# filthyrake/telescope_cam_detection

Measured on AMD Instinct MI355X. Metric: frames_per_sec, higher is better.
Workload: dtype f16x3; 1 GPU; RT-DETR-R50 640x640 bs=8/GPU, uint8 BGR frames resident in HBM -> [8,300,6] detections in HBM; synthetic seeded weights; global_batch=8, parallelism=camera-shard x1, streams_per_gpu=1, batches_in_flight_per_gpu=1, hip_graph=True

## Files before the change

### telescope_cam_detection_amd/csrc/common.h

```cpp
#pragma once
#include <hip/hip_runtime.h>
#include <stdint.h>
#include <string.h>

#include <stdexcept>
#include <string>
#include <tuple>
#include <type_traits>
#include <utility>
#include <vector>

#include "error.h"

namespace rtd {

enum DType : int { BF16 = 0, F32 = 1, U8 = 2, I32 = 3, F16X2 = 4 };
constexpr int SPLIT_GROUP = 32;
enum Act : int { ACT_NONE = 0, ACT_RELU = 1, ACT_SILU = 2, ACT_GELU = 3, ACT_LRELU = 4  };
enum ResMode : int { RES_NONE = 0, RES_PRE = 1, RES_POST = 2 };
enum DecMethod : int { DEC_DEFAULT = 0, DEC_DISCRETE = 1 };

inline size_t dtype_size(int dt) { return dt == BF16 ? 2 : (dt == U8 ? 1 : 4); }

typedef __bf16 bf16;
// ... 67 lines not shown
template <typename... KArgs, typename... Args>
inline void rtd_launch(void (*kernel)(KArgs...), dim3 grid, dim3 block, unsigned shmem, hipStream_t s, Args&&... args) {
  static_assert(sizeof...(KArgs) == sizeof...(Args), "rtd_launch: argument count differs from the kernel's parameter count");
  ++t_launches;
  if (GraphBuild* gb = t_graph_build) {
    std::tuple<std::remove_cv_t<KArgs>...> vals{static_cast<KArgs>(std::forward<Args>(args))...};
    void* ptrs[sizeof...(KArgs) + 1];
    std::apply([&](auto&... v) { size_t i = 0; ((ptrs[i++] = (void*)&v), ...); (void)i; }, vals);
    gb->add_kernel((void*)kernel, grid, block, shmem, ptrs, s);
  } else {
    hipLaunchKernelGGL(kernel, grid, block, shmem, s, static_cast<KArgs>(std::forward<Args>(args))...);
  }
}

struct ConvOpts {
  int conv_mode = 0;
  int glds_min_blocks = 4;
  int glds_min_n = 128;
  int ws2_min_blocks = 257;
  int ws64_max_blocks = 160;
  int reg_epilogue = 1;
  int conv_reg = 3;
  int prefetch = 1;
  int split_ws2_min_blocks = 257;
  int split_ws64_max_blocks = 160;
  int split_flex = 1;
  int split_flex_min_nk = 4;
  int split_flex_small_max = 200;
  int split_sx = 3;
  int split_k2 = 1;
  int split_wsq = 1;
  int split_wsq_min_blocks = 257;
  int split_wsq_min_nk = 24;
};
ConvOpts& conv_opts_template();
bool conv_set_option(const char* name, int value);

struct ConvWorkspace {
  float* slab = nullptr;
  size_t slab_bytes = 0;
};

struct ConvArgs {
  Tensor x;
  const void* w;
  const float* bias;
  Tensor res;
  Tensor x2;
  int x_up2 = 0;
  const void* next_w = nullptr;
  const float* next_bias = nullptr;
  Tensor next_y;
  int next_kpad = 0, next_act = ACT_NONE;
  Tensor avg_y;
  int y_dead = 0;
  int prefer256 = 0;
  const ConvOpts* opts = nullptr;
  Tensor y;
  int KH = 1, KW = 1, stride = 1, pad = 0;
  int Kpad = 0, Npad = 0;
  int act = ACT_NONE, res_mode = RES_NONE;
  ConvWorkspace ws;
  const void* pf = nullptr;
  size_t pf_bytes = 0;
};
void launch_conv(const ConvArgs& a, hipStream_t s);
// ... 21 lines not shown
                      float eps, hipStream_t s);
void launch_add(const Tensor& a, const Tensor& b, const Tensor& y, hipStream_t s);
void launch_axpby(float alpha, const Tensor& a, const Tensor& b, const Tensor& y, hipStream_t s);
void launch_maxpool3x3s2(const Tensor& x, const Tensor& y, hipStream_t s);
void launch_upsample2x(const Tensor& x, const Tensor& y, hipStream_t s);
void launch_avgpool2(const Tensor& x, const Tensor& y, hipStream_t s);
void launch_attention(const Tensor& qk, const Tensor& v, const Tensor& o, int heads, hipStream_t s);
void launch_set_rows(const Tensor& y, const int32_t* rows, int nrows, int rows_per_image, const float* vec,
                     hipStream_t s);
void launch_rowmax(const Tensor& x, float* out, hipStream_t s);
void launch_topk(const float* keys, int B, int N, int K, int32_t* idx, float* vals, hipStream_t s);
void launch_gather_rows(const Tensor& src, const int32_t* idx, int rows_per_image, const Tensor& dst, hipStream_t s);
void launch_ref_init(const Tensor& boxdelta, const float* anchors, const int32_t* idx, int S, float* ref_unact8,
                     float* ref8, hipStream_t s);
void launch_msdeform(const Tensor& value, int value_coff, const Tensor& offaw, const float* ref8, const Tensor& out,
                     int heads, int hd, int n_levels, int n_points, const int32_t* level_hw_start, float offset_scale,
                     int method, hipStream_t s);
void launch_box_refine(const Tensor& delta, float* ref8, hipStream_t s);
void launch_postprocess_scores(const Tensor& logits, float* scores, hipStream_t s);
bool postprocess_fused_supported(const Tensor& logits, int B, int Q);
void launch_postprocess_fused(const Tensor& logits, const float* ref8, const float* scale_wh, int B, int Q, float* block6, hipStream_t s);
void launch_postprocess_gather(const float* topv, const int32_t* topi, const float* ref8, const float* scale_wh,
                               int B, int Q, int C, float* block6, hipStream_t s);
constexpr int RTD_MAX_BATCH = 64;
struct FrameArgs {
  const uint8_t* ptr[RTD_MAX_BATCH];
  float scale_wh[2 * RTD_MAX_BATCH];
  int n;
};
void launch_preprocess_identity(const FrameArgs& fa, int H, int W, const Tensor& y, float* scale_wh_dev, hipStream_t s);
void launch_set_scale(const FrameArgs& fa, float* scale_wh_dev, hipStream_t s);
void launch_set_frame_table(const FrameArgs& fa, const uint8_t** table_dev, float* scale_wh_dev, hipStream_t s);
void launch_stem0_u8(const uint8_t* const* table_dev, int n, int H, int W, const void* w, int Kpad, const float* bias, const Tensor& y, int act,
                     hipStream_t s);
struct ResizeCoef {
  const int32_t* hb;
  const int32_t* hk;
  const int32_t* vb;
  const int32_t* vk;
  int hks, vks;
};
void launch_resize_pil(const uint8_t* src, int sh, int sw, uint8_t* tmp, const Tensor& y, int image, const ResizeCoef& coef,
                       hipStream_t s);
void launch_u8_hwc_to_chw_f32(const uint8_t* src, int H, int W, float* out, hipStream_t s);
void launch_resize_pil_u8(const uint8_t* src, int sh, int sw, uint8_t* tmp, uint8_t* dst, int dh, int dw, const ResizeCoef& c, hipStream_t s);
struct DecLin {
  const float* w;
  const float* b;
  int ldw, N, K;
};
struct DecLN {
  const float* g;
  const float* b;
};

struct DecArgs {
  int mode;
  int attn_split;
  int split;
  int B, Q, D, heads, S, n_levels, n_points, ffn, C;
  float offset_scale;
  int method;
  const float* q_in;
  const float* kfrag_in;
  const float* vfrag_in;
  const float* hs_in;
  float* hs_out;
// ... 143 lines not shown
```

### telescope_cam_detection_amd/csrc/conv_igemm.hip

```cpp
#include <stdlib.h>
#include <string.h>

#include <algorithm>
#include <type_traits>

#include "common.h"

namespace rtd {

struct ConvK {
  const void* x = nullptr;
  const void* w = nullptr;
  const float* bias = nullptr;
  const void* res = nullptr;
  void* y = nullptr;
  int M = 0, H = 0, W = 0, Cin = 0;
  long long ldx = 0, x_bstride = 0;
  int OH = 0, OW = 0, OHW = 0;
  int N = 0, Kreal = 0, Kpad = 0;
  int KH = 1, KW = 1, stride = 1, pad = 0;
  long long ldy = 0, y_bstride = 0, ldr = 0, r_bstride = 0;
  int act = ACT_NONE, res_mode = RES_NONE, y_f32 = 0, res_f32 = 0;
  int ntn = 1;
  const void* pf = nullptr;
// ... 1690 lines not shown
    const long long rpix = (long long)b * a.r_bstride + (long long)p * a.ldr;
    if (a.res_split) split_load8((const sp16*)a.res, rpix, c, rv);
    else {
      const f32x4 t0 = *(const f32x4*)((const float*)a.res + rpix + c), t1 = *(const f32x4*)((const float*)a.res + rpix + c + 4);
#pragma unroll
      for (int e = 0; e < 4; ++e) { rv[e] = t0[e]; rv[4 + e] = t1[e]; }
    }
  }
#pragma unroll
  for (int e = 0; e < 8; ++e) {
    if (a.res_mode == RES_PRE) v[e] += rv[e];
    v[e] = act_fn(v[e], a.act);
    if (a.res_mode == RES_POST) v[e] += rv[e];
  }
  if (a.y_split) split_store8((sp16*)a.y, ypix, c, v);
  else {
    *(f32x4*)((float*)a.y + ypix + c) = f32x4{v[0], v[1], v[2], v[3]};
    *(f32x4*)((float*)a.y + ypix + c + 4) = f32x4{v[4], v[5], v[6], v[7]};
  }
}

static ConvOpts g_conv_opts;
ConvOpts& conv_opts_template() { return g_conv_opts; }
bool conv_set_option(const char* name, int value) {
  ConvOpts& o = g_conv_opts;
  const struct { const char* n; int* p; } table[] = {
      {"conv_mode", &o.conv_mode}, {"glds_min_blocks", &o.glds_min_blocks}, {"glds_min_n", &o.glds_min_n},
      {"ws2_min_blocks", &o.ws2_min_blocks}, {"ws64_max_blocks", &o.ws64_max_blocks},
      {"reg_epilogue", &o.reg_epilogue}, {"conv_reg", &o.conv_reg},
      {"prefetch", &o.prefetch},
      {"split_ws2_min_blocks", &o.split_ws2_min_blocks}, {"split_ws64_max_blocks", &o.split_ws64_max_blocks},
      {"split_flex", &o.split_flex}, {"split_flex_min_nk", &o.split_flex_min_nk}, {"split_flex_small_max", &o.split_flex_small_max},
      {"split_sx", &o.split_sx}, {"split_k2", &o.split_k2}, {"split_wsq", &o.split_wsq}, {"split_wsq_min_blocks", &o.split_wsq_min_blocks},
      {"split_wsq_min_nk", &o.split_wsq_min_nk},
  };
  for (const auto& t : table)
    if (strcmp(name, t.n) == 0) { *t.p = value; return true; }
  return false;
}
static inline const ConvOpts& opts_of(const ConvArgs& a) { return a.opts ? *a.opts : g_conv_opts; }

static constexpr long long DESC_LIMIT = 1ll << 31;
static constexpr long long TILE_LIMIT = 1ll << 30;

static long long span_bytes(const Tensor& t, long long elem_bytes) {
  return ((long long)(t.n - 1) * t.bstride + ((long long)t.h * t.w - 1) * t.ld + t.c) * elem_bytes;
}

struct ConvGeom {
  int up;
  int OH, OW;
  long long M;
  bool dual;
  int K;
  explicit ConvGeom(const ConvArgs& a)
      : up(a.x_up2 ? 2 : 1), OH((a.x.h * up + 2 * a.pad - a.KH) / a.stride + 1), OW((a.x.w * up + 2 * a.pad - a.KW) / a.stride + 1),
        M((long long)a.x.n * OH * OW), dual(a.x2.p != nullptr), K(a.KH * a.KW * a.x.c + (dual ? a.x2.c : 0)) {}
};

struct RegTiles {
  int tx, ty;
  long long n;
  RegTiles(const Tensor& x, int tw) : tx((x.w + tw - 1) / tw), ty((x.h + 7) / 8), n((long long)x.n * tx * ty) {}
};

static ConvK make_convk(const ConvArgs& a, const ConvGeom& g, const ConvOpts& o) {
  const Tensor& x = a.x;
// ... 549 lines not shown
```

### telescope_cam_detection_amd/csrc/engine.hip

```cpp
#include "engine_internal.h"

using namespace rtd;
using namespace rtd_eng;

namespace rtd {
__thread GraphBuild* t_graph_build = nullptr;
__thread long long t_launches = 0;
}

void launch_force_idx(int32_t* dst, const int32_t* src, const int32_t* flag, int n, hipStream_t s);

namespace rtd_eng {
PlanOpts g_opts;
}

namespace rtd_eng {

void parse_blob(rtd_engine* e) {
  const char* b = e->blob.data();
  const size_t n = e->blob.size();
  RTD_CHECK(n >= 12 && memcmp(b, "RTDW", 4) == 0, RTD_E_WEIGHTS, "weight blob: bad magic");
  uint32_t ver, count;
  memcpy(&ver, b + 4, 4);
  memcpy(&count, b + 8, 4);
// ... 441 lines not shown
  };
  void stem(Flow& F);
  void backbone_stage(Flow& F, int si, int cin);
  void shortcut(Flow& F, Block& b);
  void bottleneck_body(Flow& F, const StageBufs& sb, const Block& b);
  void basic_body(Flow& F, const StageBufs& sb, const Block& b);
  Tensor aifi_fused(const Tensor& t0), aifi_by_op(const Tensor& t0);
  Tensor csp(const std::string& pfx, const Tensor& cat, const std::string& oname, const Tensor* up_src = nullptr);
  Tensor encoder(Flow& F);
  bool dec_fused() const {
    return e->opts.dec_fused && c.d_model == 256 && c.dec_heads == 8 && c.dec_ffn <= 1024 && c.dec_ffn % 64 == 0 && c.num_classes <= 512 &&
           c.n_levels == 3 && c.n_points >= 2 && c.n_points <= 4;
  }
  Queries select_queries(Flow& F, const Tensor& mem);
  Decoded decoder(Flow& F, const Tensor& mem, const Queries& q);
  Tensor decoder_fused(Flow& F, const Queries& q, const Tensor& vall, float* ref8, float* ref_unact8);
  Tensor decoder_by_op(const Queries& q, const Tensor& vall, const Tensor& ref8t, float* ref_unact8);
  void post_process(const Decoded& d);
};

void Builder::stem(Flow& F) {
  const int H = c.input_h, W = c.input_w;
  Tensor x = act(SP ? F32 : P, n, H, W, 8, "input");
  plan->input = x;
  const int eh = c.embedding_size / 2;
  const int h = down2(H), w = down2(W);
  Tensor s0 = act(P, n, h, w, eh);
  plan->stem_fused = SP && e->opts.stem_fused_split && eh == 32;
  if (plan->stem_fused) {
    const uint8_t** table = (const uint8_t**)alloc((size_t)c.max_batch * sizeof(void*));
    plan->frame_table = table;
    if (!dry) {
      ConvFilter w0 = get_weight(e, {{"backbone.stem.0", 9 * 8}}, P, eh);
      const void* wp = w0.w; const float* bp = w0.bias; const int kp = w0.Kpad; const int n = this->n;
      push("backbone.stem.0", "conv_igemm", 2.0 * n * h * w * eh * 27.0, (double)n * H * W * 3 + tbytes(s0),
           [table, n, H, W, wp, kp, bp, s0](hipStream_t st) { launch_stem0_u8(table, n, H, W, wp, kp, bp, s0, ACT_RELU, st); });
    }
  } else {
    conv("backbone.stem.0", x, s0, {.k = 3, .stride = 2, .pad = 1, .act = ACT_RELU, .real_cin = 3});
  }
  Tensor s1 = act(P, n, h, w, eh);
  conv("backbone.stem.1", s0, s1, {.k = 3, .pad = 1, .act = ACT_RELU});
  const Tensor s2v = mk(nullptr, P, n, h, w, c.embedding_size);
  const int ph = down2(h), pw = down2(w);
  const ConvSpec stem2{.k = 3, .pad = 1, .act = ACT_RELU};
  const long long pool_tiles = (long long)n * ((w + 31) / 32) * ((h + 7) / 8);
  const bool fuse = SP && e->opts.stem_pool_fuse && conv_pool_supported(probe(s1, s2v, stem2), probe_shape(mk(nullptr, P, n, ph, pw, c.embedding_size), 1)) &&
                    pool_tiles * 8192 < (1ll << 31);
  F.h = ph; F.w = pw;
  if (fuse) {
    F.cur = act(P, n, ph, pw, c.embedding_size, "stem");
    const ConvArgs a = args(s1, s2v, stem2, get_weight(e, {{"backbone.stem.2", 9 * s1.c}}, P, c.embedding_size, dry));
    void* side = alloc(conv_pool_side_bytes(a));
    const Tensor curv = F.cur;
    push("backbone.stem.2+pool", "conv_igemm", 2.0 * s2v.pixels() * s2v.c * 9.0 * s1.c, tbytes(s1) + tbytes(curv),
         [a, curv, side](hipStream_t st) { launch_conv_pool(a, curv, side, st); });
  } else {
    Tensor s2 = act(P, n, h, w, c.embedding_size);
    conv("backbone.stem.2", s1, s2, stem2);
    F.cur = act(P, n, ph, pw, c.embedding_size, "stem");
    const Tensor curv = F.cur;
    push("backbone.pool", "maxpool", 9.0 * curv.pixels() * curv.c, tbytes(s2) + tbytes(curv),
         [s2, curv](hipStream_t s) { launch_maxpool3x3s2(s2, curv, s); });
  }
}

void Builder::backbone_stage(Flow& F, int si, int cin) {
  const int cout = c.hidden_sizes[si];
  const bool bottleneck = c.layer_type == RTD_LAYER_BOTTLENECK;
// ... 1067 lines not shown
```

### telescope_cam_detection_amd/csrc/ops.hip

```cpp
#include <float.h>

#include <algorithm>

#include "common.h"

namespace rtd {

template <typename T> __device__ __forceinline__ float ldf(const T* p) { return (float)(*p); }
template <typename T> __device__ __forceinline__ void stf(T* p, float v) { *p = (T)v; }

__device__ __forceinline__ float wave_sum(float v) { return wave_sum64(v); }

static inline unsigned blocks_for(int64_t n, int per_block) { return (unsigned)((n + per_block - 1) / per_block); }

template <typename... KArgs, typename... Args>
static void launch_1d(void (*kernel)(KArgs...), int64_t total, hipStream_t s, Args&&... args) {
  rtd_launch(kernel, dim3(blocks_for(total, 256)), dim3(256), 0, s, std::forward<Args>(args)...);
  HIP_CHECK(hipGetLastError());
}

template <typename T> struct TypeTag { typedef T type; };
template <typename Tag> using type_of = typename Tag::type;
template <typename F>
static void with_dtype(int dt, F&& f) {
// ... 1092 lines not shown
    o[2] = (T)((float)v[0] / 255.0f);
#pragma unroll
    for (int q = 3; q < 8; ++q) o[q] = (T)0.f;
  }
}
void launch_resize_pil(const uint8_t* src, int sh, int sw, uint8_t* tmp, const Tensor& y, int image, const ResizeCoef& c,
                       hipStream_t s) {
  const int dh = y.h, dw = y.w;
  RTD_CHECK(y.c == 8 && y.ld == 8 && image < y.n, 1, "resize: output must be [n,H,W,8]");
  launch_1d(k_resize_h, (int64_t)sh * dw, s, src, sh, sw, tmp, dw, c);
  char* yp = (char*)y.p + (size_t)image * y.bstride * dtype_size(y.dt);
  with_dtype(y.dt, [&](auto t) { typedef type_of<decltype(t)> T; launch_1d(k_resize_v<T>, (int64_t)dh * dw, s, tmp, sh, dw, (T*)yp, dh, c); });
}
void launch_resize_pil_u8(const uint8_t* src, int sh, int sw, uint8_t* tmp, uint8_t* dst, int dh, int dw, const ResizeCoef& c, hipStream_t s) {
  launch_1d(k_resize_h, (int64_t)sh * dw, s, src, sh, sw, tmp, dw, c);
  launch_1d(k_resize_v<uint8_t>, (int64_t)dh * dw, s, tmp, sh, dw, dst, dh, c);
}

__global__ void k_u8_hwc_to_chw_f32(const uint8_t* __restrict__ src, int H, int W, float* __restrict__ out) {
  const int64_t i = (int64_t)blockIdx.x * blockDim.x + threadIdx.x;
  const int64_t hw = (int64_t)H * W;
  if (i >= hw) return;
  const uint8_t* px = src + i * 3;
  out[i] = (float)px[2] / 255.0f;
  out[hw + i] = (float)px[1] / 255.0f;
  out[2 * hw + i] = (float)px[0] / 255.0f;
}
void launch_u8_hwc_to_chw_f32(const uint8_t* src, int H, int W, float* out, hipStream_t s) {
  launch_1d(k_u8_hwc_to_chw_f32, (int64_t)H * W, s, src, H, W, out);
}

typedef float f32x16_s __attribute__((ext_vector_type(16)));
typedef float f32x4_s __attribute__((ext_vector_type(4)));
__global__ __launch_bounds__(256) void stem0_u8_kernel(const uint8_t* const* __restrict__ table, int H, int W, const sp16* __restrict__ wq, int Kpad,
                                                        const float* __restrict__ bias, sp16* __restrict__ y, long long y_bstride, long long ldy,
                                                        int OH, int OW, int tiles_x, int tiles_y, int act) {
  constexpr bool SPLIT = true;
  typedef sp16 E;
  typedef E Ex8 __attribute__((ext_vector_type(8)));
  typedef E Ex4 __attribute__((ext_vector_type(4)));
  constexpr int TH = 8, TW = 32, PR = 2 * TH + 1, PC = 2 * TW + 1, ROWE = 200;
  constexpr int NDW = (PC * 3 + 3 + 3) / 4;
  constexpr int ROWO = (SPLIT ? 128 : 64) + 16;
  __shared__ __attribute__((aligned(16))) E patch[PR * ROWE];
  __shared__ __attribute__((aligned(16))) E patch_lo[SPLIT ? PR * ROWE : 8];
  __shared__ __attribute__((aligned(16))) char stage[4][32 * ROWO];
  const int tid = threadIdx.x, lane = tid & 63, wv = tid >> 6, h = lane >> 5;
  int t = blockIdx.x;
  const int tx = t % tiles_x; t /= tiles_x;
  const int ty = t % tiles_y;
  const int b = t / tiles_y;
  const int x0 = tx * TW, y0 = ty * TH;
  const uint8_t* __restrict__ f = table[b];
  const long long fbytes = (long long)H * W * 3;
  const bool aligned4 = (((uintptr_t)f) & 3) == 0;
  for (int e = tid; e < PR * NDW; e += 256) {
    const int r = e / NDW, d = e - r * NDW;
    const int iy = 2 * y0 - 1 + r;
    const long long g0 = ((long long)iy * W + (2 * x0 - 1)) * 3;
    const long long a0 = (g0 & ~3ll) + 4ll * d;
    unsigned dw = 0;
    const bool row_ok = (unsigned)iy < (unsigned)H;
    if (row_ok) {
      if (aligned4 && a0 >= 0 && a0 + 4 <= fbytes) dw = *(const unsigned*)(f + a0);
      else {
#pragma unroll
        for (int q = 0; q < 4; ++q)
          if (a0 + q >= 0 && a0 + q < fbytes) dw |= (unsigned)f[a0 + q] << (8 * q);
      }
    }
#pragma unroll
    for (int q = 0; q < 4; ++q) {
      const int el = (int)(a0 + q - g0);
      if (el < 0 || el >= PC * 3) continue;
      const int ix = 2 * x0 - 1 + el / 3;
      const float v = (row_ok && (unsigned)ix < (unsigned)W) ? (float)((dw >> (8 * q)) & 0xffu) : 0.f;
      const float vn = v / 255.0f;
      const E hi = (E)vn;
      patch[r * ROWE + el] = hi;
      if (SPLIT) patch_lo[r * ROWE + el] = (E)(vn - (float)hi);
    }
  }
  for (int e = tid; e < PR * (ROWE - PC * 3); e += 256) {
    const int r = e / (ROWE - PC * 3), i = e - r * (ROWE - PC * 3);
    patch[r * ROWE + PC * 3 + i] = (E)0.f;
    if (SPLIT) patch_lo[r * ROWE + PC * 3 + i] = (E)0.f;
  }
  Ex8 wf[2], wfl[2];
  int doff[2][4];
#pragma unroll
  for (int s = 0; s < 2; ++s) {
#pragma unroll
    for (int j = 0; j < 8; ++j) {
      const int k = 16 * s + 8 * h + j;
      const int kh = k / 10, e = k - kh * 10;
      const int kw = e / 3, cb = e - kw * 3;
      const int kr = (kh * 3 + kw) * 8 + (2 - cb);
      const bool real = k < 30 && e < 9;
      if (SPLIT) {
        const size_t pos = (size_t)(lane & 31) * Kpad + ((kr >> 5) << 6) + (kr & 31);
        wf[s][j] = real ? wq[pos] : (E)0.f;
        wfl[s][j] = real ? wq[pos + 32] : (E)0.f;
      } else {
        wf[s][j] = real ? wq[(size_t)(lane & 31) * Kpad + kr] : (E)0.f;
      }
    }
#pragma unroll
    for (int j = 0; j < 4; ++j) {
      const int k = 16 * s + 8 * h + 2 * j;
      const int kh = k / 10, e = k - kh * 10;
      doff[s][j] = k < 30 ? kh * ROWE + e : 0;
    }
  }
  __syncthreads();
#pragma unroll 1
  for (int rr = 0; rr < 2; ++rr) {
    const int r = wv * 2 + rr;
    const int eoff = (2 * r) * ROWE + (2 * (lane & 31)) * 3;
    const E* base = patch + eoff;
    f32x16_s acc;
#pragma unroll
    for (int e = 0; e < 16; ++e) acc[e] = 0.f;
#pragma unroll
    for (int s = 0; s < 2; ++s) {
      typedef unsigned u4_s __attribute__((ext_vector_type(4)));
      unsigned xd[4];
#pragma unroll
      for (int j = 0; j < 4; ++j) xd[j] = *(const unsigned*)(base + doff[s][j]);
      const u4_s xv = {xd[0], xd[1], xd[2], xd[3]};
      if constexpr (SPLIT) acc = mfma_pair32(wf[s], __builtin_bit_cast(Ex8, xv), acc);
      else acc = __builtin_amdgcn_mfma_f32_32x32x16_bf16(wf[s], __builtin_bit_cast(Ex8, xv), acc, 0, 0, 0);
      if constexpr (SPLIT) {
        unsigned xl[4];
#pragma unroll
        for (int j = 0; j < 4; ++j) xl[j] = *(const unsigned*)(patch_lo + eoff + doff[s][j]);
        const u4_s xlv = {xl[0], xl[1], xl[2], xl[3]};
        acc = mfma_pair32(wf[s], __builtin_bit_cast(Ex8, xlv), acc);
        acc = mfma_pair32(wfl[s], __builtin_bit_cast(Ex8, xv), acc);
      }
    }
    const int oy = y0 + r;
    char* sw_ = stage[wv];
#pragma unroll
    for (int q = 0; q < 4; ++q) {
      const f32x4_s bv = *(const f32x4_s*)(bias + 8 * q + 4 * h);
      Ex4 o, ol;
#pragma unroll
      for (int e = 0; e < 4; ++e) {
        float v = acc[4 * q + e] + bv[e];
        if (act == ACT_RELU) v = fmaxf(v, 0.f);
        else if (act == ACT_SILU) v = v / (1.f + __expf(-v));
        if constexpr (SPLIT) { sp16 hh, ll; split2(v, hh, ll); o[e] = hh; ol[e] = ll; }
        else o[e] = (E)v;
      }
      *(Ex4*)(sw_ + (lane & 31) * ROWO + (8 * q + 4 * h) * 2) = o;
      if (SPLIT) *(Ex4*)(sw_ + (lane & 31) * ROWO + 64 + (8 * q + 4 * h) * 2) = ol;
    }
    __builtin_amdgcn_wave_barrier();
    if (oy < OH) {
      constexpr int CPP = SPLIT ? 8 : 4;
      E* yrow = y + (SPLIT ? 2 : 1) * ((long long)b * y_bstride + ((long long)oy * OW + x0) * ldy);
#pragma unroll
      for (int i2 = 0; i2 < CPP / 2; ++i2) {
        const int idx = i2 * 64 + lane;
        const int p = idx / CPP, ch = idx % CPP;
        if (x0 + p < OW) *(Ex8*)(yrow + (SPLIT ? 2 : 1) * (long long)p * ldy + ch * 8) = *(const Ex8*)(sw_ + p * ROWO + ch * 16);
      }
    }
    __builtin_amdgcn_wave_barrier();
  }
}
void launch_stem0_u8(const uint8_t* const* table_dev, int n, int H, int W, const void* w, int Kpad, const float* bias, const Tensor& y, int act,
                     hipStream_t s) {
  const int OH = (H + 2 - 3) / 2 + 1, OW = (W + 2 - 3) / 2 + 1;
  RTD_CHECK(y.dt == F16X2 && y.c == 32 && y.h == OH && y.w == OW && y.n >= n && y.ld % SPLIT_GROUP == 0 &&
                (act == ACT_RELU || act == ACT_NONE || act == ACT_SILU), 1, "stem0_u8: output must be F16X2 [n, H/2, W/2, 32]");
  const int tiles_x = (OW + 31) / 32, tiles_y = (OH + 7) / 8;
  rtd_launch(stem0_u8_kernel, dim3((unsigned)(n * tiles_x * tiles_y)), dim3(256), 0, s, table_dev, H, W, (const sp16*)w, Kpad, bias, (sp16*)y.p,
                     (long long)y.bstride, (long long)y.ld, OH, OW, tiles_x, tiles_y, act);
  HIP_CHECK(hipGetLastError());
}

struct CropNorm { float mean[3], inv_std[3]; };
__global__ void k_crop_resize(const CropBatch cb, int n, int S, CropNorm nm, float* __restrict__ out) {
  const int64_t i = (int64_t)blockIdx.x * blockDim.x + threadIdx.x;
  const int64_t per = (int64_t)S * S;
  if (i >= per * n) return;
  const int c = (int)(i / per);
  const int p = (int)(i - (int64_t)c * per);
  const int oy = p / S, ox = p - oy * S;
  const int cw = cb.x2[c] - cb.x1[c], chh = cb.y2[c] - cb.y1[c];
  const float sx = (float)cw / (float)S, sy = (float)chh / (float)S;
  const float fx = fmaxf(sx * ((float)ox + 0.5f) - 0.5f, 0.f), fy = fmaxf(sy * ((float)oy + 0.5f) - 0.5f, 0.f);
  const int x0 = min((int)fx, cw - 1), y0 = min((int)fy, chh - 1);
  const int x1 = min(x0 + 1, cw - 1), y1 = min(y0 + 1, chh - 1);
  const float lx1 = fx - (float)x0, ly1 = fy - (float)y0, lx0 = 1.f - lx1, ly0 = 1.f - ly1;
  const uint8_t* f = cb.frame[c];
  const int64_t fw = cb.fw[c];
  const uint8_t* p00 = f + ((int64_t)(cb.y1[c] + y0) * fw + cb.x1[c] + x0) * 3;
  const uint8_t* p01 = f + ((int64_t)(cb.y1[c] + y0) * fw + cb.x1[c] + x1) * 3;
  const uint8_t* p10 = f + ((int64_t)(cb.y1[c] + y1) * fw + cb.x1[c] + x0) * 3;
  const uint8_t* p11 = f + ((int64_t)(cb.y1[c] + y1) * fw + cb.x1[c] + x1) * 3;
#pragma unroll
  for (int ch = 0; ch < 3; ++ch) {
    const int sc = 2 - ch;
    const float v = ly0 * (lx0 * (float)p00[sc] + lx1 * (float)p01[sc]) + ly1 * (lx0 * (float)p10[sc] + lx1 * (float)p11[sc]);
    out[((int64_t)c * 3 + ch) * per + p] = (v / 255.0f - nm.mean[ch]) * nm.inv_std[ch];
  }
}
void launch_crop_resize(const CropBatch& cb, int n, int out_size, const float mean[3], const float stdv[3], float* out, hipStream_t s) {
  RTD_CHECK(n >= 1 && n <= 64 && out_size >= 1 && out_size <= 4096, 1, "crop batch: 1..64 crops per launch");
  for (int i = 0; i < n; ++i) {
// ... 11 lines not shown
```

### telescope_cam_detection_amd/csrc/testapi.hip

```cpp
#include "engine_internal.h"

using namespace rtd;
using namespace rtd_eng;

using backend::OpScratch;
static bool rows_fit_int(int a, int b) { return a >= 1 && b >= 1 && (int64_t)a * b <= 0x7fffffff; }
static Tensor rows_view(const void* p, int dt, int n, int rows, int c, int64_t ld) {
  Tensor t = mk(p, dt, n, rows, 1, c);
  t.ld = ld; t.bstride = (int64_t)rows * ld;
  return t;
}

extern "C" {

int rtd_debug_tensor(rtd_handle h, const char* name, float* out, int64_t capacity, int64_t shape[4]) {
  return guarded(h, [&] {
    RTD_CHECK(name && shape && h->last_n > 0, RTD_E_STATE, "no forward has run");
    Plan* p = h->plans[h->last_n].get();
    auto it = p->named.find(name);
    RTD_CHECK(it != p->named.end(), RTD_E_INVALID, std::string("unknown debug tensor ") + name);
    const Tensor& t = it->second;
    if (p->stem_fused && strcmp(name, "input") == 0 && out) {
      HIP_CHECK(hipSetDevice(h->cfg.device));
      launch_preprocess_identity(h->last_fa, h->cfg.input_h, h->cfg.input_w, p->input, p->scale_wh, h->q.stream);
// ... 261 lines not shown
    }
    a.avg_y = mk(avg_y, F16X2, B, H / 2, W / 2, Cout);
    a.y_dead = y_dead;
    RTD_CHECK(conv_avg_supported(a) && conv_sx_batch_fits(a), RTD_E_INVALID, "conv + average: shape not taken by the streaming kernel");
    give_slab(sc, a);
    launch_conv(a, nullptr);
    HIP_CHECK(hipDeviceSynchronize());
  });
}

int rtd_op_conv_pool(const void* x, const void* w_ohwi_f32, const float* bias, void* pooled, int B, int H, int W) {
  if (!x || !w_ohwi_f32 || !bias || !pooled) return RTD_E_INVALID;
  return op_guard([&] {
    RTD_CHECK(B >= 1 && H >= 1 && W >= 1, RTD_E_INVALID, "conv + max-pool: extents");
    OpScratch sc;
    const ConvFilter f = dev_filter(sc, F16X2, w_ohwi_f32, bias, 64, 9 * 32);
    const ConvArgs a = conv_args(mk(x, F16X2, B, H, W, 32), mk(nullptr, F16X2, B, H, W, 64), f, 3, 1, 1, ACT_RELU);
    const Tensor p = mk(pooled, F16X2, B, H / 2, W / 2, 64);
    RTD_CHECK(conv_pool_supported(a, p), RTD_E_INVALID, "conv + max-pool: shape not supported (even extents, >= 32 tiles of 8 x 32 per image, conv_reg)");
    launch_conv_pool(a, p, sc.get<char>(conv_pool_side_bytes(a)), nullptr);
    HIP_CHECK(hipDeviceSynchronize());
  });
}

int rtd_op_stem0_u8(const uint8_t* const* frames_dev, int n, int H, int W, const void* w_ohwi_f32, const float* bias, void* y, int act) {
  if (!frames_dev || !w_ohwi_f32 || !bias || !y || n < 1 || n > RTD_MAX_BATCH || H < 1 || W < 1) return RTD_E_INVALID;
  if (act != ACT_NONE && act != ACT_RELU && act != ACT_SILU) return RTD_E_INVALID;
  for (int i = 0; i < n; ++i)
    if (!frames_dev[i]) return RTD_E_INVALID;
  return op_guard([&] {
    OpScratch sc;
    const ConvFilter f = dev_filter(sc, F16X2, w_ohwi_f32, bias, 32, 9 * 8);
    const uint8_t* const* table = sc.upload(frames_dev, (size_t)n);
    launch_stem0_u8(table, n, H, W, f.w, f.Kpad, f.bias, mk(y, F16X2, n, (H - 1) / 2 + 1, (W - 1) / 2 + 1, 32), act, nullptr);
    HIP_CHECK(hipDeviceSynchronize());
  });
}

static void report_out(const ConvChoiceReport& r, char* key, int key_capacity, int32_t* info) {
  RTD_CHECK(key && info && key_capacity > (int)strlen(r.key), RTD_E_INVALID, "conv choice: key buffer too small");
  strcpy(key, r.key);
  const int v[12] = {r.family, r.stages, r.bn, r.mt, r.bm, r.smallc, r.wsq, r.sx, r.cog, r.S, r.grid, r.ntn};
  for (int i = 0; i < 12; ++i) info[i] = v[i];
}
int rtd_debug_conv_choice(int dtype, int B, int H, int W, int Cin, int C2, int Cout, int KH, int stride, int pad, int res_mode, int out_f32,
                          int x_up2, int Cnext, int avg, int pool, char* key, int key_capacity, int32_t* info) {
  return backend::caught(create_error(), [&] {
    RTD_CHECK(dtype == BF16 || dtype == F32 || dtype == F16X2, RTD_E_INVALID, "conv choice: dtype");
    RTD_CHECK(B >= 1 && H >= 1 && W >= 1 && Cin >= 1 && C2 >= 0 && Cout >= 1 && KH >= 1 && stride >= 1 && pad >= 0 && Cnext >= 0, RTD_E_INVALID, "conv choice: extents");
    RTD_CHECK(!x_up2 || !((H | W) & 1), RTD_E_INVALID, "conv choice: x_up2 needs even output extents");
    const void* const P = (const void*)(uintptr_t)4096;
    const int OH = (H + 2 * pad - KH) / stride + 1, OW = (W + 2 * pad - KH) / stride + 1;
    ConvFilter f = conv_filter_extents(dtype, Cout, KH * KH * Cin + C2);
    f.w = (void*)P; f.bias = (float*)P;
    ConvArgs a = conv_args(x_up2 ? mk(P, dtype, B, H / 2, W / 2, Cin) : mk(P, dtype, B, H, W, Cin), mk(P, out_f32 ? F32 : dtype, B, OH, OW, Cout), f, KH, stride, pad,
                           ACT_RELU);
    a.x_up2 = x_up2;
    a.res_mode = res_mode;
    if (res_mode != RES_NONE) a.res = mk(P, dtype, B, OH, OW, Cout);
    if (C2) a.x2 = mk(P, dtype, B, OH, OW, C2);
    if (Cnext) {
      a.next_w = P; a.next_bias = (const float*)P; a.next_y = mk(P, dtype, B, OH, OW, Cnext);
      a.next_kpad = conv_filter_extents(dtype, Cnext, Cout).Kpad; a.next_act = ACT_RELU;
    }
    if (avg) a.avg_y = mk(P, dtype, B, OH / 2, OW / 2, Cout);
    ConvChoiceReport r;
    if (pool) {
// ... 369 lines not shown
```

Before: 1682 frames/s.

## Make stem0 u8 conv persistent with double-buffered patch prefetch and LDS weights

Turns the first stem conv kernel, which reads raw uint8 frames, into a persistent kernel with a grid capped at a few blocks per CU. Each block loops over tiles and issues the global loads for the next tile before running the MFMA compute on the current one, using double-buffered LDS patches. It also caches the filter in LDS, builds a 256-entry lookup table for the u8 to split-f16 conversion, hoists the bias loads, and templates the activation. The cost is more LDS per block, which may lower occupancy, and a new tunable grid cap option.

```diff
diff --git a/telescope_cam_detection_amd/csrc/common.h b/telescope_cam_detection_amd/csrc/common.h
--- a/telescope_cam_detection_amd/csrc/common.h
+++ b/telescope_cam_detection_amd/csrc/common.h
@@ -123,6 +123,7 @@
   int split_wsq = 1;
   int split_wsq_min_blocks = 257;
   int split_wsq_min_nk = 24;
+  int stem0_grid = 0;
 };
 ConvOpts& conv_opts_template();
 bool conv_set_option(const char* name, int value);
@@ -210,7 +211,7 @@
 void launch_set_scale(const FrameArgs& fa, float* scale_wh_dev, hipStream_t s);
 void launch_set_frame_table(const FrameArgs& fa, const uint8_t** table_dev, float* scale_wh_dev, hipStream_t s);
 void launch_stem0_u8(const uint8_t* const* table_dev, int n, int H, int W, const void* w, int Kpad, const float* bias, const Tensor& y, int act,
-                     hipStream_t s);
+                     int grid_cap, hipStream_t s);
 struct ResizeCoef {
   const int32_t* hb;
   const int32_t* hk;
diff --git a/telescope_cam_detection_amd/csrc/conv_igemm.hip b/telescope_cam_detection_amd/csrc/conv_igemm.hip
--- a/telescope_cam_detection_amd/csrc/conv_igemm.hip
+++ b/telescope_cam_detection_amd/csrc/conv_igemm.hip
@@ -1746,7 +1746,7 @@
       {"split_ws2_min_blocks", &o.split_ws2_min_blocks}, {"split_ws64_max_blocks", &o.split_ws64_max_blocks},
       {"split_flex", &o.split_flex}, {"split_flex_min_nk", &o.split_flex_min_nk}, {"split_flex_small_max", &o.split_flex_small_max},
       {"split_sx", &o.split_sx}, {"split_k2", &o.split_k2}, {"split_wsq", &o.split_wsq}, {"split_wsq_min_blocks", &o.split_wsq_min_blocks},
-      {"split_wsq_min_nk", &o.split_wsq_min_nk},
+      {"split_wsq_min_nk", &o.split_wsq_min_nk}, {"stem0_grid", &o.stem0_grid},
   };
   for (const auto& t : table)
     if (strcmp(name, t.n) == 0) { *t.p = value; return true; }
diff --git a/telescope_cam_detection_amd/csrc/engine.hip b/telescope_cam_detection_amd/csrc/engine.hip
--- a/telescope_cam_detection_amd/csrc/engine.hip
+++ b/telescope_cam_detection_amd/csrc/engine.hip
@@ -497,9 +497,9 @@
     plan->frame_table = table;
     if (!dry) {
       ConvFilter w0 = get_weight(e, {{"backbone.stem.0", 9 * 8}}, P, eh);
-      const void* wp = w0.w; const float* bp = w0.bias; const int kp = w0.Kpad; const int n = this->n;
+      const void* wp = w0.w; const float* bp = w0.bias; const int kp = w0.Kpad; const int n = this->n, cap = e->conv_opts.stem0_grid;
       push("backbone.stem.0", "conv_igemm", 2.0 * n * h * w * eh * 27.0, (double)n * H * W * 3 + tbytes(s0),
-           [table, n, H, W, wp, kp, bp, s0](hipStream_t st) { launch_stem0_u8(table, n, H, W, wp, kp, bp, s0, ACT_RELU, st); });
+           [table, n, H, W, wp, kp, bp, s0, cap](hipStream_t st) { launch_stem0_u8(table, n, H, W, wp, kp, bp, s0, ACT_RELU, cap, st); });
     }
   } else {
     conv("backbone.stem.0", x, s0, {.k = 3, .stride = 2, .pad = 1, .act = ACT_RELU, .real_cin = 3});
diff --git a/telescope_cam_detection_amd/csrc/ops.hip b/telescope_cam_detection_amd/csrc/ops.hip
--- a/telescope_cam_detection_amd/csrc/ops.hip
+++ b/telescope_cam_detection_amd/csrc/ops.hip
@@ -1148,60 +1148,52 @@
 
 typedef float f32x16_s __attribute__((ext_vector_type(16)));
 typedef float f32x4_s __attribute__((ext_vector_type(4)));
+constexpr int STEM0_BLOCKS_PER_CU = 3;
+template <int ACT>
 __global__ __launch_bounds__(256) void stem0_u8_kernel(const uint8_t* const* __restrict__ table, int H, int W, const sp16* __restrict__ wq, int Kpad,
                                                         const float* __restrict__ bias, sp16* __restrict__ y, long long y_bstride, long long ldy,
-                                                        int OH, int OW, int tiles_x, int tiles_y, int act) {
-  constexpr bool SPLIT = true;
+                                                        int OH, int OW, int tiles_x, int tiles_y, int ntiles) {
   typedef sp16 E;
   typedef E Ex8 __attribute__((ext_vector_type(8)));
   typedef E Ex4 __attribute__((ext_vector_type(4)));
+  typedef unsigned short u16;
   constexpr int TH = 8, TW = 32, PR = 2 * TH + 1, PC = 2 * TW + 1, ROWE = 200;
   constexpr int NDW = (PC * 3 + 3 + 3) / 4;
-  constexpr int ROWO = (SPLIT ? 128 : 64) + 16;
-  __shared__ __attribute__((aligned(16))) E patch[PR * ROWE];
-  __shared__ __attribute__((aligned(16))) E patch_lo[SPLIT ? PR * ROWE : 8];
+  constexpr int NSLOT = (PR * NDW + 255) / 256;
+  constexpr int ROWO = 128 + 16;
+  constexpr int DUMP = PR * ROWE;
+  __shared__ __attribute__((aligned(16))) u16 patch[2][PR * ROWE + 8];
+  __shared__ __attribute__((aligned(16))) u16 patch_lo[2][PR * ROWE + 8];
   __shared__ __attribute__((aligned(16))) char stage[4][32 * ROWO];
+  __shared__ unsigned pairtab[256];
   const int tid = threadIdx.x, lane = tid & 63, wv = tid >> 6, h = lane >> 5;
-  int t = blockIdx.x;
-  const int tx = t % tiles_x; t /= tiles_x;
-  const int ty = t % tiles_y;
-  const int b = t / tiles_y;
-  const int x0 = tx * TW, y0 = ty * TH;
-  const uint8_t* __restrict__ f = table[b];
   const long long fbytes = (long long)H * W * 3;
-  const bool aligned4 = (((uintptr_t)f) & 3) == 0;
-  for (int e = tid; e < PR * NDW; e += 256) {
-    const int r = e / NDW, d = e - r * NDW;
-    const int iy = 2 * y0 - 1 + r;
-    const long long g0 = ((long long)iy * W + (2 * x0 - 1)) * 3;
-    const long long a0 = (g0 & ~3ll) + 4ll * d;
-    unsigned dw = 0;
-    const bool row_ok = (unsigned)iy < (unsigned)H;
-    if (row_ok) {
-      if (aligned4 && a0 >= 0 && a0 + 4 <= fbytes) dw = *(const unsigned*)(f + a0);
-      else {
-#pragma unroll
-        for (int q = 0; q < 4; ++q)
-          if (a0 + q >= 0 && a0 + q < fbytes) dw |= (unsigned)f[a0 + q] << (8 * q);
-      }
-    }
-#pragma unroll
-    for (int q = 0; q < 4; ++q) {
-      const int el = (int)(a0 + q - g0);
-      if (el < 0 || el >= PC * 3) continue;
-      const int ix = 2 * x0 - 1 + el / 3;
-      const float v = (row_ok && (unsigned)ix < (unsigned)W) ? (float)((dw >> (8 * q)) & 0xffu) : 0.f;
-      const float vn = v / 255.0f;
-      const E hi = (E)vn;
-      patch[r * ROWE + el] = hi;
-      if (SPLIT) patch_lo[r * ROWE + el] = (E)(vn - (float)hi);
-    }
-  }
-  for (int e = tid; e < PR * (ROWE - PC * 3); e += 256) {
-    const int r = e / (ROWE - PC * 3), i = e - r * (ROWE - PC * 3);
-    patch[r * ROWE + PC * 3 + i] = (E)0.f;
-    if (SPLIT) patch_lo[r * ROWE + PC * 3 + i] = (E)0.f;
-  }
+  const int per_image = tiles_x * tiles_y;
+
+  {
+    const float vn = (float)tid / 255.0f;
+    const E hi = (E)vn, lo = (E)(vn - (float)hi);
+    pairtab[tid] = (unsigned)__builtin_bit_cast(u16, hi) | ((unsigned)__builtin_bit_cast(u16, lo) << 16);
+  }
+  E* wl = (E*)&stage[0][0];
+  for (int c = tid; c < 32 * Kpad / 8; c += 256) ((Ex8*)wl)[c] = ((const Ex8*)wq)[c];
+  for (int e = tid; e < 2 * PR * (ROWE - PC * 3); e += 256) {
+    const int bf = e / (PR * (ROWE - PC * 3)), e1 = e - bf * (PR * (ROWE - PC * 3));
+    const int r = e1 / (ROWE - PC * 3), i = e1 - r * (ROWE - PC * 3);
+    patch[bf][r * ROWE + PC * 3 + i] = 0;
+    patch_lo[bf][r * ROWE + PC * 3 + i] = 0;
+  }
+  int srow[NSLOT], sdw[NSLOT];
+#pragma unroll
+  for (int i = 0; i < NSLOT; ++i) {
+    const int e = tid + 256 * i;
+    srow[i] = e < PR * NDW ? e / NDW : 0;
+    sdw[i] = e < PR * NDW ? e - (e / NDW) * NDW : NDW;
+  }
+  f32x4_s bv[4];
+#pragma unroll
+  for (int q = 0; q < 4; ++q) bv[q] = *(const f32x4_s*)(bias + 8 * q + 4 * h);
+  __syncthreads();
   Ex8 wf[2], wfl[2];
   int doff[2][4];
 #pragma unroll
@@ -1213,13 +1205,9 @@
       const int kw = e / 3, cb = e - kw * 3;
       const int kr = (kh * 3 + kw) * 8 + (2 - cb);
       const bool real = k < 30 && e < 9;
-      if (SPLIT) {
-        const size_t pos = (size_t)(lane & 31) * Kpad + ((kr >> 5) << 6) + (kr & 31);
-        wf[s][j] = real ? wq[pos] : (E)0.f;
-        wfl[s][j] = real ? wq[pos + 32] : (E)0.f;
-      } else {
-        wf[s][j] = real ? wq[(size_t)(lane & 31) * Kpad + kr] : (E)0.f;
-      }
+      const int pos = (lane & 31) * Kpad + ((kr >> 5) << 6) + (kr & 31);
+      wf[s][j] = real ? wl[pos] : (E)0.f;
+      wfl[s][j] = real ? wl[pos + 32] : (E)0.f;
     }
 #pragma unroll
     for (int j = 0; j < 4; ++j) {
@@ -1228,72 +1216,146 @@
       doff[s][j] = k < 30 ? kh * ROWE + e : 0;
     }
   }
-  __syncthreads();
-#pragma unroll 1
-  for (int rr = 0; rr < 2; ++rr) {
-    const int r = wv * 2 + rr;
-    const int eoff = (2 * r) * ROWE + (2 * (lane & 31)) * 3;
-    const E* base = patch + eoff;
-    f32x16_s acc;
-#pragma unroll
-    for (int e = 0; e < 16; ++e) acc[e] = 0.f;
-#pragma unroll
-    for (int s = 0; s < 2; ++s) {
-      typedef unsigned u4_s __attribute__((ext_vector_type(4)));
-      unsigned xd[4];
-#pragma unroll
-      for (int j = 0; j < 4; ++j) xd[j] = *(const unsigned*)(base + doff[s][j]);
-      const u4_s xv = {xd[0], xd[1], xd[2], xd[3]};
-      if constexpr (SPLIT) acc = mfma_pair32(wf[s], __builtin_bit_cast(Ex8, xv), acc);
-      else acc = __builtin_amdgcn_mfma_f32_32x32x16_bf16(wf[s], __builtin_bit_cast(Ex8, xv), acc, 0, 0, 0);
-      if constexpr (SPLIT) {
-        unsigned xl[4];
-#pragma unroll
-        for (int j = 0; j < 4; ++j) xl[j] = *(const unsigned*)(patch_lo + eoff + doff[s][j]);
+
+  typedef const __attribute__((address_space(1))) uint8_t* GBytes;
+  typedef const __attribute__((address_space(1))) unsigned* GWord;
+  auto request = [&](int b, int y0, int x0, unsigned (&raw)[NSLOT]) {
+    const uint8_t* fp = table[b];
+    const GBytes f = (GBytes)fp;
+    const bool aligned4 = (((uintptr_t)fp) & 3) == 0;
+#pragma unroll
+    for (int i = 0; i < NSLOT; ++i) {
+      const int iy = 2 * y0 - 1 + srow[i];
+      const bool ok = sdw[i] < NDW && (unsigned)iy < (unsigned)H;
+      const long long g0 = ((long long)iy * W + (2 * x0 - 1)) * 3;
+      const long long a0 = (g0 & ~3ll) + 4ll * sdw[i];
+      unsigned dw = 0;
+      if (aligned4 && a0 >= 0 && a0 + 4 <= fbytes) {
+        if (ok) dw = *(GWord)(f + a0);
+      } else {
+#pragma unroll
+        for (int q = 0; q < 4; ++q) {
+          const bool in = ok && a0 + q >= 0 && a0 + q < fbytes;
+          const unsigned v = f[in ? a0 + q : 0];
+          dw |= in ? v << (8 * q) : 0u;
+        }
+      }
+      raw[i] = dw;
+    }
+  };
+  auto convert = [&](int y0, int x0, const unsigned (&raw)[NSLOT], u16* __restrict__ ph, u16* __restrict__ pl) {
+    const int el_lo = max(0, 3 * (1 - 2 * x0)), el_hi_row = min(PC * 3, 3 * (W + 1 - 2 * x0));
+#pragma unroll
+    for (int i = 0; i < NSLOT; ++i) {
+      const int iy = 2 * y0 - 1 + srow[i];
+      const int phase = (int)((((unsigned)iy * (unsigned)W + (unsigned)(2 * x0 - 1)) * 3u) & 3u);
+      const int el_hi = (unsigned)iy < (unsigned)H ? el_hi_row : 0;
+      const int el0 = 4 * sdw[i] - phase;
+#pragma unroll
+      for (int q = 0; q < 4; ++q) {
+        const int el = el0 + q;
+        const unsigned pr = pairtab[(el >= el_lo && el < el_hi) ? ((raw[i] >> (8 * q)) & 0xffu) : 0u];
+        const int at = (unsigned)el < (unsigned)(PC * 3) ? srow[i] * ROWE + el : DUMP;
+        ph[at] = (u16)pr;
+        pl[at] = (u16)(pr >> 16);
+      }
+    }
+  };
+  auto compute = [&](int b, int y0, int x0, const u16* __restrict__ ph, const u16* __restrict__ pl) {
+#pragma unroll
+    for (int rr = 0; rr < 2; ++rr) {
+      const int r = wv * 2 + rr;
+      const int eoff = (2 * r) * ROWE + (2 * (lane & 31)) * 3;
+      f32x16_s acc;
+#pragma unroll
+      for (int e = 0; e < 16; ++e) acc[e] = 0.f;
+#pragma unroll
+      for (int s = 0; s < 2; ++s) {
+        typedef unsigned u4_s __attribute__((ext_vector_type(4)));
+        unsigned xd[4], xl[4];
+#pragma unroll
+        for (int j = 0; j < 4; ++j) xd[j] = *(const unsigned*)(ph + eoff + doff[s][j]);
+#pragma unroll
+        for (int j = 0; j < 4; ++j) xl[j] = *(const unsigned*)(pl + eoff + doff[s][j]);
+        const u4_s xv = {xd[0], xd[1], xd[2], xd[3]};
         const u4_s xlv = {xl[0], xl[1], xl[2], xl[3]};
+        acc = mfma_pair32(wf[s], __builtin_bit_cast(Ex8, xv), acc);
         acc = mfma_pair32(wf[s], __builtin_bit_cast(Ex8, xlv), acc);
         acc = mfma_pair32(wfl[s], __builtin_bit_cast(Ex8, xv), acc);
       }
-    }
-    const int oy = y0 + r;
-    char* sw_ = stage[wv];
-#pragma unroll
-    for (int q = 0; q < 4; ++q) {
-      const f32x4_s bv = *(const f32x4_s*)(bias + 8 * q + 4 * h);
-      Ex4 o, ol;
-#pragma unroll
-      for (int e = 0; e < 4; ++e) {
-        float v = acc[4 * q + e] + bv[e];
-        if (act == ACT_RELU) v = fmaxf(v, 0.f);
-        else if (act == ACT_SILU) v = v / (1.f + __expf(-v));
-        if constexpr (SPLIT) { sp16 hh, ll; split2(v, hh, ll); o[e] = hh; ol[e] = ll; }
-        else o[e] = (E)v;
-      }
-      *(Ex4*)(sw_ + (lane & 31) * ROWO + (8 * q + 4 * h) * 2) = o;
-      if (SPLIT) *(Ex4*)(sw_ + (lane & 31) * ROWO + 64 + (8 * q + 4 * h) * 2) = ol;
-    }
-    __builtin_amdgcn_wave_barrier();
-    if (oy < OH) {
-      constexpr int CPP = SPLIT ? 8 : 4;
-      E* yrow = y + (SPLIT ? 2 : 1) * ((long long)b * y_bstride + ((long long)oy * OW + x0) * ldy);
+      const int oy = y0 + r;
+      char* sw_ = stage[wv];
+#pragma unroll
+      for (int q = 0; q < 4; ++q) {
+        Ex4 o, ol;
+#pragma unroll
+        for (int e = 0; e < 4; ++e) {
+          float v = acc[4 * q + e] + bv[q][e];
+          if constexpr (ACT == ACT_RELU) v = fmaxf(v, 0.f);
+          else if constexpr (ACT == ACT_SILU) v = v / (1.f + __expf(-v));
+          sp16 hh, ll;
+          split2(v, hh, ll);
+          o[e] = hh; ol[e] = ll;
+        }
+        *(Ex4*)(sw_ + (lane & 31) * ROWO + (8 * q + 4 * h) * 2) = o;
+        *(Ex4*)(sw_ + (lane & 31) * ROWO + 64 + (8 * q + 4 * h) * 2) = ol;
+      }
+      __builtin_amdgcn_wave_barrier();
+      constexpr int CPP = 8;
+      E* yrow = y + 2 * ((long long)b * y_bstride + ((long long)oy * OW + x0) * ldy);
 #pragma unroll
       for (int i2 = 0; i2 < CPP / 2; ++i2) {
         const int idx = i2 * 64 + lane;
         const int p = idx / CPP, ch = idx % CPP;
-        if (x0 + p < OW) *(Ex8*)(yrow + (SPLIT ? 2 : 1) * (long long)p * ldy + ch * 8) = *(const Ex8*)(sw_ + p * ROWO + ch * 16);
-      }
-    }
-    __builtin_amdgcn_wave_barrier();
-  }
+        if (oy < OH && x0 + p < OW) *(Ex8*)(yrow + 2 * (long long)p * ldy + ch * 8) = *(const Ex8*)(sw_ + p * ROWO + ch * 16);
+      }
+      __builtin_amdgcn_wave_barrier();
+    }
+  };
+  auto locate = [&](int t, int& b, int& y0, int& x0) {
+    b = t / per_image;
+    const int r = t - b * per_image, ty = r / tiles_x;
+    y0 = ty * TH; x0 = (r - ty * tiles_x) * TW;
+  };
+
+  int b, y0, x0, buf = 0;
+  unsigned raw[NSLOT];
+  locate(blockIdx.x, b, y0, x0);
+  request(b, y0, x0, raw);
+  convert(y0, x0, raw, patch[0], patch_lo[0]);
+  __syncthreads();
+#pragma unroll 1
+  for (int tn = blockIdx.x + gridDim.x; tn < ntiles; tn += gridDim.x, buf ^= 1) {
+    int bn, y0n, x0n;
+    locate(tn, bn, y0n, x0n);
+    request(bn, y0n, x0n, raw);
+    compute(b, y0, x0, patch[buf], patch_lo[buf]);
+    convert(y0n, x0n, raw, patch[buf ^ 1], patch_lo[buf ^ 1]);
+    __syncthreads();
+    b = bn; y0 = y0n; x0 = x0n;
+  }
+  compute(b, y0, x0, patch[buf], patch_lo[buf]);
 }
 void launch_stem0_u8(const uint8_t* const* table_dev, int n, int H, int W, const void* w, int Kpad, const float* bias, const Tensor& y, int act,
-                     hipStream_t s) {
+                     int grid_cap, hipStream_t s) {
   const int OH = (H + 2 - 3) / 2 + 1, OW = (W + 2 - 3) / 2 + 1;
   RTD_CHECK(y.dt == F16X2 && y.c == 32 && y.h == OH && y.w == OW && y.n >= n && y.ld % SPLIT_GROUP == 0 &&
                 (act == ACT_RELU || act == ACT_NONE || act == ACT_SILU), 1, "stem0_u8: output must be F16X2 [n, H/2, W/2, 32]");
+  RTD_CHECK(Kpad % 8 == 0 && Kpad <= 288 && ((uintptr_t)w & 15) == 0, 1, "stem0_u8: the filter rows must fit the kernel's LDS copy");
   const int tiles_x = (OW + 31) / 32, tiles_y = (OH + 7) / 8;
-  rtd_launch(stem0_u8_kernel, dim3((unsigned)(n * tiles_x * tiles_y)), dim3(256), 0, s, table_dev, H, W, (const sp16*)w, Kpad, bias, (sp16*)y.p,
-                     (long long)y.bstride, (long long)y.ld, OH, OW, tiles_x, tiles_y, act);
+  const long long ntiles = (long long)n * tiles_x * tiles_y;
+  RTD_CHECK(ntiles < (1ll << 30), 1, "stem0_u8: too many tiles");
+  int dev = 0, cus = 0;
+  HIP_CHECK(hipGetDevice(&dev));
+  HIP_CHECK(hipDeviceGetAttribute(&cus, hipDeviceAttributeMultiprocessorCount, dev));
+  const long long want = grid_cap > 0 ? grid_cap : (long long)STEM0_BLOCKS_PER_CU * std::max(cus, 1);
+  auto go = [&](auto kernel) {
+    rtd_launch(kernel, dim3((unsigned)std::min(ntiles, want)), dim3(256), 0, s, table_dev, H, W, (const sp16*)w, Kpad, bias, (sp16*)y.p,
+               (long long)y.bstride, (long long)y.ld, OH, OW, tiles_x, tiles_y, (int)ntiles);
+  };
+  if (act == ACT_RELU) go(stem0_u8_kernel<ACT_RELU>);
+  else if (act == ACT_SILU) go(stem0_u8_kernel<ACT_SILU>);
+  else go(stem0_u8_kernel<ACT_NONE>);
   HIP_CHECK(hipGetLastError());
 }
 
diff --git a/telescope_cam_detection_amd/csrc/testapi.hip b/telescope_cam_detection_amd/csrc/testapi.hip
--- a/telescope_cam_detection_amd/csrc/testapi.hip
+++ b/telescope_cam_detection_amd/csrc/testapi.hip
@@ -317,7 +317,8 @@
     OpScratch sc;
     const ConvFilter f = dev_filter(sc, F16X2, w_ohwi_f32, bias, 32, 9 * 8);
     const uint8_t* const* table = sc.upload(frames_dev, (size_t)n);
-    launch_stem0_u8(table, n, H, W, f.w, f.Kpad, f.bias, mk(y, F16X2, n, (H - 1) / 2 + 1, (W - 1) / 2 + 1, 32), act, nullptr);
+    launch_stem0_u8(table, n, H, W, f.w, f.Kpad, f.bias, mk(y, F16X2, n, (H - 1) / 2 + 1, (W - 1) / 2 + 1, 32), act,
+                    conv_opts_template().stem0_grid, nullptr);
     HIP_CHECK(hipDeviceSynchronize());
   });
 }
```

Result: no change. 1688 frames/s, median of 6 (+0.4%).
